# ZeningLin/ViBERTgrid-PyTorch

Hardware: AMD Instinct MI355X
Metric: training docs/sec, 512x512 img + seq_len 512, bert-base+resnet34; 1/2/4/8 GPU (higher is better)
Workload: dtype f32

## Files before the change

vibertgrid-pytorch_amd/csrc/gemm_planes.hip:

```cpp
#include "vbg_common.h"
#include <type_traits>
#include <cstdlib>
#include <hip/hip_ext.h>
#include "../../include/vbg.h"

namespace vbg {

typedef unsigned pg_u32x4 __attribute__((ext_vector_type(4)));
typedef __bf16 pg_bf16x8 __attribute__((ext_vector_type(8)));
constexpr unsigned PG_INVALID = 0x80000000u;

__device__ __forceinline__ __amdgpu_buffer_rsrc_t pg_rsrc(const void* base) {
    return __builtin_amdgcn_make_buffer_rsrc(const_cast<void*>(base), 0, (int)0x80000000u, 0x00020000);
}

typedef _Float16 pg_f16x8 __attribute__((ext_vector_type(8)));
__device__ __forceinline__ void pg_split2(float a, float b, unsigned& hi, unsigned& lo) {
    typedef float f32x2_t __attribute__((ext_vector_type(2)));
    typedef _Float16 f16x2_t __attribute__((ext_vector_type(2)));
    const f32x2_t v = {a, b};
    const f16x2_t h = __builtin_convertvector(v, f16x2_t);
    const f16x2_t l = __builtin_convertvector((v - __builtin_convertvector(h, f32x2_t)) * 2048.f, f16x2_t);
    hi = __builtin_bit_cast(unsigned, h);
    lo = __builtin_bit_cast(unsigned, l);
// ... 386 lines not shown
        if (gm >= M || gn >= N) continue;
        float4 v = *reinterpret_cast<const float4*>(&Ct[row * CTS + c]);
        if (add_bias) {
            const float4 b = *reinterpret_cast<const float4*>(bias + gn);
            v.x += b.x; v.y += b.y; v.z += b.z; v.w += b.w;
        }
        float* cp = C + (long long)gm * ldc + gn;
        if (atomic) {
            unsafeAtomicAdd(cp + 0, v.x); unsafeAtomicAdd(cp + 1, v.y); unsafeAtomicAdd(cp + 2, v.z); unsafeAtomicAdd(cp + 3, v.w);
            continue;
        }
        if (accumulate) {
            const float4 o = *reinterpret_cast<const float4*>(cp);
            v.x += o.x; v.y += o.y; v.z += o.z; v.w += o.w;
        }
        if (epi == VBG_EPI_RELU) v = make_float4(fmaxf(v.x, 0.f), fmaxf(v.y, 0.f), fmaxf(v.z, 0.f), fmaxf(v.w, 0.f));
        if (epi == VBG_EPI_MUL_GELU_GRAD) {
            const float4 hv = *reinterpret_cast<const float4*>(C2 + (long long)gm * ldc + gn);
            v.x *= gelu_erf_grad(hv.x); v.y *= gelu_erf_grad(hv.y); v.z *= gelu_erf_grad(hv.z); v.w *= gelu_erf_grad(hv.w);
        }
        if (C) *reinterpret_cast<float4*>(cp) = v;
        vmax = fmaxf(fmaxf(vmax, fmaxf(fabsf(v.x), fabsf(v.y))), fmaxf(fabsf(v.z), fabsf(v.w)));
        if (p.colsum) *reinterpret_cast<float4*>(&Ct[row * CTS + c]) = v;
        if (epi == VBG_EPI_GELU_DUAL) {
            v = make_float4(gelu_erf(v.x), gelu_erf(v.y), gelu_erf(v.z), gelu_erf(v.w));
            if (C2) *reinterpret_cast<float4*>(C2 + (long long)gm * ldc + gn) = v;
        }
        if (Cp) {
            const float e[4] = {v.x, v.y, v.z, v.w};
            unsigned short h[4], m[4], l[4];
#pragma unroll
            for (int t = 0; t < 4; ++t) {
                const unsigned u = __float_as_uint(e[t]);
                const float r1 = e[t] - __uint_as_float(u & 0xffff0000u);
                const unsigned u1 = __float_as_uint(r1);
                const float r2 = r1 - __uint_as_float(u1 & 0xffff0000u);
                h[t] = (unsigned short)(u >> 16); m[t] = (unsigned short)(u1 >> 16); l[t] = (unsigned short)(__float_as_uint(r2) >> 16);
            }
            unsigned short* o = Cp + (long long)gm * p.ldp + gn;
            *reinterpret_cast<uint2*>(o) = make_uint2(h[0] | ((unsigned)h[1] << 16), h[2] | ((unsigned)h[3] << 16));
            *reinterpret_cast<uint2*>(o + p.c_plane) = make_uint2(m[0] | ((unsigned)m[1] << 16), m[2] | ((unsigned)m[3] << 16));
            *reinterpret_cast<uint2*>(o + 2 * p.c_plane) = make_uint2(l[0] | ((unsigned)l[1] << 16), l[2] | ((unsigned)l[3] << 16));
        }
        if (Cq) {
            unsigned short* o = Cq + (long long)gm * p.ldq + gn;
            uint2 h, l;
            pg_split2(v.x * qsc, v.y * qsc, h.x, l.x);
            pg_split2(v.z * qsc, v.w * qsc, h.y, l.y);
            *reinterpret_cast<uint2*>(o) = h;
            *reinterpret_cast<uint2*>(o + p.q_plane) = l;
        }
    }
    if (p.colsum) {
        __syncthreads();
        if (tid < BN && n0 + tid < N) {
            float cs = 0.f;
            const int rows = min(BM, M - m0);
            for (int r = 0; r < rows; ++r) cs += Ct[r * CTS + tid];
            unsafeAtomicAdd(p.colsum + n0 + tid, cs);
        }
    }
    if (p.c_amax) {
        __syncthreads();
        vbg_amax_publish(vmax, p.c_amax, Ct);
    }
}

__device__ __forceinline__ void pg_split3(float x, unsigned short& h, unsigned short& m, unsigned short& l);

__global__ __launch_bounds__(512) void plane_gemm_256_kernel(const vbg_plane_gemm_desc p) {
    constexpr int BM = 256, BN = 256, WGN = 4, NW = 8, NT = 512, NST = 3, BK = 16;
    constexpr int WM = 128, WN = 64, TM = 4, TN = 2;
    constexpr int PA = BM * 32, PB = BN * 32;
    constexpr int STAGE = 3 * (PA + PB);
    constexpr int NIA = 3, NIB = 3;
    constexpr int CTS = BN + 4;
    constexpr int SMEM = NST * STAGE;
    static_assert(64 * CTS * 4 <= SMEM, "epilogue pass fits");
    __shared__ __attribute__((aligned(1024))) unsigned char smem[SMEM];

    const int tid = threadIdx.x, lane = tid & 63, wave = tid >> 6;
    const int M = p.M, N = p.N;
    const long long a_plane = p.a_plane, b_plane = p.b_plane, lda = p.lda, ldb = p.ldb;
    constexpr unsigned XCDS = 8, XCD_GROUP = 8;
    const unsigned gx = gridDim.x, gy = gridDim.y;
    const unsigned lin = blockIdx.x + gridDim.x * blockIdx.y;
    const unsigned total = gx * gy;
    const unsigned xcd = lin % XCDS, local = lin / XCDS;
    const unsigned per_xcd = (total + XCDS - 1) / XCDS, tall = (total % XCDS) ? (total % XCDS) : XCDS;
    const unsigned rem = xcd < tall ? xcd * per_xcd + local : tall * per_xcd + (xcd - tall) * (per_xcd - 1) + local;
    const unsigned band = XCD_GROUP * gy, bid = rem / band, first = bid * XCD_GROUP;
    const unsigned bm = min(gx - first, XCD_GROUP), inb = rem - bid * band;
    const unsigned tile_m = first + inb % bm, tile_n = inb / bm;
    const int m0 = (int)tile_m * BM, n0 = (int)tile_n * BN;
    if (m0 >= M || n0 >= N) return;
    const int ntiles = p.K / BK;

    unsigned avo[NIA], bvo[NIB];
    int alds[NIA], blds[NIB];
    {
        const int lrow = lane >> 1;
#pragma unroll
        for (int i = 0; i < NIA; ++i) {
            const int u = wave + NW * i, q = u / 8, rb = u % 8;
            const int r = rb * 32 + lrow;
            const int half = (lane & 1) ^ ((r >> 3) & 1);
            avo[i] = (m0 + r < M) ? (unsigned)(((long long)q * a_plane + (long long)r * lda) * 2 + half * 16) : PG_INVALID;
            alds[i] = __builtin_amdgcn_readfirstlane(q * PA + rb * 1024);
        }
#pragma unroll
        for (int i = 0; i < NIB; ++i) {
            const int u = wave + NW * i, q = u / 8, rb = u % 8;
            const int r = rb * 32 + lrow;
            const int half = (lane & 1) ^ ((r >> 3) & 1);
            bvo[i] = (n0 + r < N) ? (unsigned)(((long long)q * b_plane + (long long)r * ldb) * 2 + half * 16) : PG_INVALID;
            blds[i] = __builtin_amdgcn_readfirstlane(3 * PA + q * PB + rb * 1024);
        }
    }
    const unsigned short* abase = p.A + (long long)m0 * lda;
    const unsigned short* bbase = p.B + (long long)n0 * ldb;
    typedef __attribute__((address_space(3))) void* lds_ptr;
    auto issue = [&](int stage, unsigned inv) {
        unsigned char* sb = smem + stage * STAGE;
        const __amdgpu_buffer_rsrc_t ra = pg_rsrc(abase), rb = pg_rsrc(bbase);
#pragma unroll
        for (int i = 0; i < NIA; ++i)
            __builtin_amdgcn_raw_ptr_buffer_load_lds(ra, (lds_ptr)(sb + alds[i]), 16, (int)(avo[i] | inv), 0, 0, 0);
#pragma unroll
        for (int i = 0; i < NIB; ++i)
            __builtin_amdgcn_raw_ptr_buffer_load_lds(rb, (lds_ptr)(sb + blds[i]), 16, (int)(bvo[i] | inv), 0, 0, 0);
        abase += BK;
        bbase += BK;
    };

    const int wm = wave / WGN, wn = wave % WGN;
    const int lr = lane & 31, lk = lane >> 5;
    const int fo = lr * 32 + ((lk ^ ((lr >> 3) & 1)) << 4);
    f32x16 acc[TM][TN];
#pragma unroll
    for (int i = 0; i < TM; ++i)
#pragma unroll
        for (int j = 0; j < TN; ++j)
#pragma unroll
            for (int r = 0; r < 16; ++r) acc[i][j][r] = 0.f;
    pg_u32x4 fa[3][TM], fb[3][TN];
    auto read_frags = [&](int stage) {
        const unsigned char* as = smem + stage * STAGE + (wm * WM) * 32 + fo;
        const unsigned char* bs = smem + stage * STAGE + 3 * PA + (wn * WN) * 32 + fo;
        constexpr int order[3] = {2, 0, 1};
#pragma unroll
        for (int o = 0; o < 3; ++o) {
            const int q = order[o];
#pragma unroll
            for (int i = 0; i < TM; ++i) fa[q][i] = *reinterpret_cast<const pg_u32x4*>(as + q * PA + i * 32 * 32);
#pragma unroll
            for (int j = 0; j < TN; ++j) fb[q][j] = *reinterpret_cast<const pg_u32x4*>(bs + q * PB + j * 32 * 32);
        }
    };
    auto mma = [&]() {
        constexpr int qa[6] = {2, 0, 1, 1, 0, 0}, qb[6] = {0, 2, 1, 0, 1, 0};
#pragma unroll
        for (int t = 0; t < 6; ++t)
#pragma unroll
            for (int i = 0; i < TM; ++i)
#pragma unroll
                for (int j = 0; j < TN; ++j)
                    acc[i][j] = __builtin_amdgcn_mfma_f32_32x32x16_bf16(__builtin_bit_cast(pg_bf16x8, fa[qa[t]][i]),
                                                                        __builtin_bit_cast(pg_bf16x8, fb[qb[t]][j]), acc[i][j], 0, 0, 0);
    };
    constexpr int NIW = NIA + NIB;
    issue(0, 0u);
    issue(1, ntiles > 1 ? 0u : PG_INVALID);
    asm volatile("s_waitcnt vmcnt(%0)" ::"n"(NIW) : "memory");
    __builtin_amdgcn_s_barrier();
    int cur = 0;
    for (int t = 0; t < ntiles; ++t) {
        const int nxt = (cur + 1 == NST) ? 0 : cur + 1;
        const int nn = (nxt + 1 == NST) ? 0 : nxt + 1;
        issue(nn, t + 2 < ntiles ? 0u : PG_INVALID);
        read_frags(cur);
        mma();
        asm volatile("s_waitcnt vmcnt(%0) lgkmcnt(0)" ::"n"(NIW) : "memory");
        __builtin_amdgcn_s_barrier();
        cur = nxt;
    }
    __syncthreads();

    const float* bias = p.bias;
    const int epi = p.epi;
    const float alpha = p.alpha;
    const long long ldc = p.ldc;
    float* const C = p.C;
    float* const C2 = p.C2;
    unsigned short* const Cp = p.Cp;
    float* const Ct = reinterpret_cast<float*>(smem);
    constexpr int QN = BN / 4;
#pragma unroll
    for (int ps = 0; ps < 4; ++ps) {
        if (wm == (ps >> 1)) {
#pragma unroll
            for (int ii = 0; ii < 2; ++ii)
#pragma unroll
                for (int j = 0; j < TN; ++j)
#pragma unroll
                    for (int r = 0; r < 16; ++r)
                        Ct[(ii * 32 + (r & 3) + 8 * (r >> 2) + 4 * lk) * CTS + wn * WN + j * 32 + lr] = acc[2 * (ps & 1) + ii][j][r] * alpha;
        }
        __syncthreads();
#pragma unroll
        for (int q = 0; q < 64 * QN / NT; ++q) {
            const int idx = tid + q * NT;
            const int row = idx / QN, c = (idx % QN) * 4;
            const int gm = m0 + ps * 64 + row, gn = n0 + c;
            if (gm >= M || gn >= N) continue;
            float4 v = *reinterpret_cast<const float4*>(&Ct[row * CTS + c]);
            if (bias) {
                const float4 b = *reinterpret_cast<const float4*>(bias + gn);
                v.x += b.x; v.y += b.y; v.z += b.z; v.w += b.w;
            }
            float* cp = C + (long long)gm * ldc + gn;
            if (epi == VBG_EPI_RELU) v = make_float4(fmaxf(v.x, 0.f), fmaxf(v.y, 0.f), fmaxf(v.z, 0.f), fmaxf(v.w, 0.f));
            if (epi == VBG_EPI_MUL_GELU_GRAD) {
                const float4 hv = *reinterpret_cast<const float4*>(C2 + (long long)gm * ldc + gn);
                v.x *= gelu_erf_grad(hv.x); v.y *= gelu_erf_grad(hv.y); v.z *= gelu_erf_grad(hv.z); v.w *= gelu_erf_grad(hv.w);
            }
            if (C) *reinterpret_cast<float4*>(cp) = v;
            if (epi == VBG_EPI_GELU_DUAL) {
                v = make_float4(gelu_erf(v.x), gelu_erf(v.y), gelu_erf(v.z), gelu_erf(v.w));
                if (C2) *reinterpret_cast<float4*>(C2 + (long long)gm * ldc + gn) = v;
            }
            if (Cp) {
                const float e[4] = {v.x, v.y, v.z, v.w};
                unsigned short h[4], m[4], l[4];
#pragma unroll
                for (int t = 0; t < 4; ++t) pg_split3(e[t], h[t], m[t], l[t]);
                unsigned short* o = Cp + (long long)gm * p.ldp + gn;
                *reinterpret_cast<uint2*>(o) = make_uint2(h[0] | ((unsigned)h[1] << 16), h[2] | ((unsigned)h[3] << 16));
                *reinterpret_cast<uint2*>(o + p.c_plane) = make_uint2(m[0] | ((unsigned)m[1] << 16), m[2] | ((unsigned)m[3] << 16));
                *reinterpret_cast<uint2*>(o + 2 * p.c_plane) = make_uint2(l[0] | ((unsigned)l[1] << 16), l[2] | ((unsigned)l[3] << 16));
            }
        }
        __syncthreads();
    }
}

__device__ __forceinline__ void pg_split3(float x, unsigned short& h, unsigned short& m, unsigned short& l) {
    const unsigned u = __float_as_uint(x);
    const float r1 = x - __uint_as_float(u & 0xffff0000u);
    const unsigned u1 = __float_as_uint(r1);
    const float r2 = r1 - __uint_as_float(u1 & 0xffff0000u);
    h = (unsigned short)(u >> 16); m = (unsigned short)(u1 >> 16); l = (unsigned short)(__float_as_uint(r2) >> 16);
}

__global__ __launch_bounds__(256) void split_planes_kernel(const float* __restrict__ x, long long ldx, int rows, int cols,
                                                            unsigned short* __restrict__ out, int ldp, long long plane, int relu,
                                                            float* colsum) {
    extern __shared__ float sh_cols[];
    const int cpr = ldp / 8;
    const long long n = (long long)rows * cpr;
    const long long stride = (long long)gridDim.x * blockDim.x;
    float cs[8] = {0.f, 0.f, 0.f, 0.f, 0.f, 0.f, 0.f, 0.f};
    const long long i0 = (long long)blockIdx.x * blockDim.x + threadIdx.x;
    for (long long i = i0; i < n; i += stride) {
        const int r = (int)(i / cpr), c = (int)(i % cpr) * 8;
        float e[8];
        if (c + 8 <= cols && ((ldx & 3) == 0) && ((((uintptr_t)x) & 15) == 0)) {
            const float4 a = *reinterpret_cast<const float4*>(x + (long long)r * ldx + c);
            const float4 b = *reinterpret_cast<const float4*>(x + (long long)r * ldx + c + 4);
            e[0] = a.x; e[1] = a.y; e[2] = a.z; e[3] = a.w; e[4] = b.x; e[5] = b.y; e[6] = b.z; e[7] = b.w;
        } else {
#pragma unroll
            for (int t = 0; t < 8; ++t) e[t] = (c + t < cols) ? x[(long long)r * ldx + c + t] : 0.f;
        }
        unsigned short h[8], m[8], l[8];
#pragma unroll
        for (int t = 0; t < 8; ++t) {
            cs[t] += e[t];
            pg_split3(relu ? fmaxf(e[t], 0.f) : e[t], h[t], m[t], l[t]);
        }
        unsigned short* o = out + (long long)r * ldp + c;
        auto pack = [](const unsigned short* s) {
            return make_uint4(s[0] | ((unsigned)s[1] << 16), s[2] | ((unsigned)s[3] << 16), s[4] | ((unsigned)s[5] << 16), s[6] | ((unsigned)s[7] << 16));
        };
        *reinterpret_cast<uint4*>(o) = pack(h);
        *reinterpret_cast<uint4*>(o + plane) = pack(m);
        *reinterpret_cast<uint4*>(o + 2 * plane) = pack(l);
    }
    if (colsum) {
        for (int c = threadIdx.x; c < ldp; c += blockDim.x) sh_cols[c] = 0.f;
        __syncthreads();
        if (i0 < n) {
            const int c = (int)(i0 % cpr) * 8;
#pragma unroll
            for (int t = 0; t < 8; ++t) atomicAdd(&sh_cols[c + t], cs[t]);
        }
        __syncthreads();
        for (int c = threadIdx.x; c < cols; c += blockDim.x) {
            const float v = sh_cols[c];
            if (v != 0.f) unsafeAtomicAdd(colsum + c, v);
        }
    }
}

__global__ __launch_bounds__(256) void split_planes_pair_kernel(const float* __restrict__ x, long long ldx, int rows, int cols,
                                                                 unsigned short* __restrict__ out, int ldp, long long plane,
                                                                 const unsigned* amax, float* colsum) {
    extern __shared__ float sh_cols[];
    const float sc = amax ? vbg_pow2_scale(vbg_amax_read(amax)).x : 1.f;
    float cs[8] = {0.f, 0.f, 0.f, 0.f, 0.f, 0.f, 0.f, 0.f};
    const long long i0 = (long long)blockIdx.x * blockDim.x + threadIdx.x;
    const int cpr = ldp / 8;
    const long long n = (long long)rows * cpr;
    const long long stride = (long long)gridDim.x * blockDim.x;
    const bool vec = ((ldx & 3) == 0) && ((((uintptr_t)x) & 15) == 0);
    for (long long i = (long long)blockIdx.x * blockDim.x + threadIdx.x; i < n; i += stride) {
        const int r = (int)(i / cpr), c = (int)(i % cpr) * 8;
        float e[8];
        if (c + 8 <= cols && vec) {
            const float4 a = *reinterpret_cast<const float4*>(x + (long long)r * ldx + c);
            const float4 b = *reinterpret_cast<const float4*>(x + (long long)r * ldx + c + 4);
            e[0] = a.x; e[1] = a.y; e[2] = a.z; e[3] = a.w; e[4] = b.x; e[5] = b.y; e[6] = b.z; e[7] = b.w;
        } else {
#pragma unroll
            for (int t = 0; t < 8; ++t) e[t] = (c + t < cols) ? x[(long long)r * ldx + c + t] : 0.f;
        }
#pragma unroll
        for (int t = 0; t < 8; ++t) { cs[t] += e[t]; e[t] *= sc; }
        uint4 h, l;
        pg_split2(e[0], e[1], h.x, l.x); pg_split2(e[2], e[3], h.y, l.y); pg_split2(e[4], e[5], h.z, l.z); pg_split2(e[6], e[7], h.w, l.w);
        unsigned short* o = out + (long long)r * ldp + c;
        *reinterpret_cast<uint4*>(o) = h;
        *reinterpret_cast<uint4*>(o + plane) = l;
    }
    if (colsum) {
        for (int c = threadIdx.x; c < ldp; c += blockDim.x) sh_cols[c] = 0.f;
        __syncthreads();
        if (i0 < n) {
            const int c = (int)(i0 % cpr) * 8;
#pragma unroll
            for (int t = 0; t < 8; ++t) atomicAdd(&sh_cols[c + t], cs[t]);
        }
        __syncthreads();
        for (int c = threadIdx.x; c < cols; c += blockDim.x) {
            const float v = sh_cols[c];
            if (v != 0.f) unsafeAtomicAdd(colsum + c, v);
        }
    }
}

__global__ __launch_bounds__(256) void col_l1_max_kernel(const vbg_l1_entry* __restrict__ tab, unsigned* __restrict__ out) {
    const vbg_l1_entry e = tab[blockIdx.y];
    const int c0 = blockIdx.x * 64;
    if (c0 >= e.cols) return;
    const int tx = threadIdx.x & 15, ty = threadIdx.x >> 4;
    const int c = c0 + tx * 4;
    const bool vec = (e.ld & 3) == 0 && ((((uintptr_t)e.w) & 15) == 0) && c + 4 <= e.cols;
    float4 s = make_float4(0.f, 0.f, 0.f, 0.f);
#pragma unroll 4
    for (int r = ty; r < e.rows; r += 16) {
        const float* p = e.w + (long long)r * e.ld + c;
        if (vec) {
            const float4 v = *reinterpret_cast<const float4*>(p);
            s.x += fabsf(v.x); s.y += fabsf(v.y); s.z += fabsf(v.z); s.w += fabsf(v.w);
        } else {
            if (c < e.cols) s.x += fabsf(p[0]);
            if (c + 1 < e.cols) s.y += fabsf(p[1]);
            if (c + 2 < e.cols) s.z += fabsf(p[2]);
            if (c + 3 < e.cols) s.w += fabsf(p[3]);
        }
    }
    __shared__ float4 red[16][16];
    red[ty][tx] = s;
    __syncthreads();
    if (ty == 0) {
        float4 t = red[0][tx];
#pragma unroll
        for (int g = 1; g < 16; ++g) { const float4 v = red[g][tx]; t.x += v.x; t.y += v.y; t.z += v.z; t.w += v.w; }
        float m = fmaxf(fmaxf(t.x, t.y), fmaxf(t.z, t.w));
#pragma unroll
        for (int o = 8; o > 0; o >>= 1) m = fmaxf(m, __shfl_xor(m, o, 64));
        if (tx == 0) atomicMax(out + blockIdx.y, __float_as_uint(m));
    }
}

__global__ __launch_bounds__(256) void split_planes_t_kernel(const float* __restrict__ x, long long ldx, int rows, int cols,
                                                              unsigned short* __restrict__ out, int ldp, long long plane) {
    __shared__ float t[64][65];
    const int r0 = blockIdx.x * 64, c0 = blockIdx.y * 64;
    const int tid = threadIdx.x;
    const bool vec = ((ldx & 3) == 0) && ((((uintptr_t)x) & 15) == 0);
#pragma unroll
    for (int i = 0; i < 4; ++i) {
        const int f = tid + i * 256, r = f / 16, c = (f % 16) * 4;
        float4 v = make_float4(0.f, 0.f, 0.f, 0.f);
        if (r0 + r < rows) {
            const float* src = x + (long long)(r0 + r) * ldx + c0 + c;
            if (vec && c0 + c + 4 <= cols) v = *reinterpret_cast<const float4*>(src);
            else {
                if (c0 + c + 0 < cols) v.x = src[0];
                if (c0 + c + 1 < cols) v.y = src[1];
                if (c0 + c + 2 < cols) v.z = src[2];
                if (c0 + c + 3 < cols) v.w = src[3];
            }
        }
        t[r][c] = v.x; t[r][c + 1] = v.y; t[r][c + 2] = v.z; t[r][c + 3] = v.w;
    }
    __syncthreads();
#pragma unroll
    for (int i = 0; i < 2; ++i) {
        const int f = tid + i * 256, c = f / 8, rg = (f % 8) * 8;
        if (c0 + c >= cols || r0 + rg >= ldp) continue;
        unsigned short h[8], m[8], l[8];
#pragma unroll
        for (int e = 0; e < 8; ++e) pg_split3(t[rg + e][c], h[e], m[e], l[e]);
        unsigned short* o = out + (long long)(c0 + c) * ldp + r0 + rg;
        auto pack = [](const unsigned short* s) {
            return make_uint4(s[0] | ((unsigned)s[1] << 16), s[2] | ((unsigned)s[3] << 16), s[4] | ((unsigned)s[5] << 16), s[6] | ((unsigned)s[7] << 16));
        };
        *reinterpret_cast<uint4*>(o) = pack(h);
        *reinterpret_cast<uint4*>(o + plane) = pack(m);
        *reinterpret_cast<uint4*>(o + 2 * plane) = pack(l);
    }
}

template <bool PAIR>
__global__ __launch_bounds__(256) void split_planes_t_batched_kernel(const float* __restrict__ src, unsigned short* __restrict__ dst,
                                                                      const long long* __restrict__ tbl, int njobs, long long plane) {
    __shared__ float t[64][65];
    int j = 0;
    while (j + 1 < njobs && (long long)blockIdx.x >= tbl[(j + 1) * 6 + 5]) ++j;
    const long long* e = tbl + j * 6;
    const float* x = src + e[0];
    const int rows = (int)e[1], cols = (int)e[2], ldp = (int)e[4];
    unsigned short* out = dst + e[3];
    const int local = (int)(blockIdx.x - e[5]);
    const int tr = (ldp + 63) / 64;
    const int r0 = (local % tr) * 64, c0 = (local / tr) * 64;
    const int tid = threadIdx.x;
    const long long ldx = cols;
#pragma unroll
    for (int i = 0; i < 4; ++i) {
        const int f = tid + i * 256, r = f / 16, c = (f % 16) * 4;
        float v[4] = {0.f, 0.f, 0.f, 0.f};
        if (r0 + r < rows) {
#pragma unroll
            for (int q = 0; q < 4; ++q)
                if (c0 + c + q < cols) v[q] = x[(long long)(r0 + r) * ldx + c0 + c + q];
        }
        t[r][c] = v[0]; t[r][c + 1] = v[1]; t[r][c + 2] = v[2]; t[r][c + 3] = v[3];
    }
    __syncthreads();
#pragma unroll
    for (int i = 0; i < 2; ++i) {
        const int f = tid + i * 256, c = f / 8, rg = (f % 8) * 8;
        if (c0 + c >= cols || r0 + rg >= ldp) continue;
        unsigned short* o = out + (long long)(c0 + c) * ldp + r0 + rg;
        if constexpr (PAIR) {
            uint4 h, l;
            pg_split2(t[rg + 0][c], t[rg + 1][c], h.x, l.x); pg_split2(t[rg + 2][c], t[rg + 3][c], h.y, l.y);
            pg_split2(t[rg + 4][c], t[rg + 5][c], h.z, l.z); pg_split2(t[rg + 6][c], t[rg + 7][c], h.w, l.w);
            *reinterpret_cast<uint4*>(o) = h;
            *reinterpret_cast<uint4*>(o + plane) = l;
            continue;
        }
        unsigned short h[8], m[8], l[8];
#pragma unroll
        for (int q = 0; q < 8; ++q) pg_split3(t[rg + q][c], h[q], m[q], l[q]);
        auto pack = [](const unsigned short* s) {
            return make_uint4(s[0] | ((unsigned)s[1] << 16), s[2] | ((unsigned)s[3] << 16), s[4] | ((unsigned)s[5] << 16), s[6] | ((unsigned)s[7] << 16));
        };
        *reinterpret_cast<uint4*>(o) = pack(h);
        *reinterpret_cast<uint4*>(o + plane) = pack(m);
        *reinterpret_cast<uint4*>(o + 2 * plane) = pack(l);
    }
}

template <int BM, int BN, int WGM, int WGN, int NST, bool TRANS = false, int FORM = 1>
static void pg_launch_pair(const vbg_plane_gemm_desc& d, hipStream_t s, hipEvent_t e0, hipEvent_t e1) {
    dim3 g(cdiv(d.M, BM), cdiv(d.N, BN), 1);
    if (d.ngroups > 0) {
        int total = 0;
        for (int i = 0; i < d.ngroups; ++i) total += d.grp[i].tiles_m * d.grp[i].tiles_n;
        g = dim3(total, 1, 1);
    }
    (void)hipGetLastError();
    if (e0 && e1) hipExtLaunchKernelGGL((plane_gemm_kernel<BM, BN, WGM, WGN, NST, TRANS, FORM>), g, dim3(WGM * WGN * 64), 0, s, e0, e1, 0, d);
    else hipLaunchKernelGGL((plane_gemm_kernel<BM, BN, WGM, WGN, NST, TRANS, FORM>), g, dim3(WGM * WGN * 64), 0, s, d);
}

template <int BM, int BN, int WGM, int WGN, int NST, bool TRANS = false>
static void pg_launch(const vbg_plane_gemm_desc& d, hipStream_t s, hipEvent_t e0, hipEvent_t e1) {
    dim3 g(cdiv(d.M, BM), cdiv(d.N, BN), d.splitk);
    if (d.ngroups > 0) {
        int total = 0;
        for (int i = 0; i < d.ngroups; ++i) total += d.grp[i].tiles_m * d.grp[i].tiles_n;
        g = dim3(total, 1, d.splitk);
    }
    (void)hipGetLastError();
    if (e0 && e1) hipExtLaunchKernelGGL((plane_gemm_kernel<BM, BN, WGM, WGN, NST, TRANS>), g, dim3(WGM * WGN * 64), 0, s, e0, e1, 0, d);
    else hipLaunchKernelGGL((plane_gemm_kernel<BM, BN, WGM, WGN, NST, TRANS>), g, dim3(WGM * WGN * 64), 0, s, d);
}

}

using namespace vbg;

static int plane_gemm_dispatch(const vbg_plane_gemm_desc* desc, void* stream, void* e0, void* e1) {
    VBG_CHECK_ARG(desc != nullptr);
    vbg_plane_gemm_desc d = *desc;
    if (d.ngroups > 0) {
        VBG_CHECK_ARG(d.ngroups <= VBG_PLANE_MAX_GROUPS && d.Cp == nullptr && d.bias == nullptr && d.C2 == nullptr);
        for (int i = 0; i < d.ngroups; ++i) {
            vbg_plane_group& g = d.grp[i];
            VBG_CHECK_ARG(g.A && g.B && g.C && g.M > 0 && g.N > 0 && g.N % 4 == 0 && g.ldc % 4 == 0 && ((uintptr_t)g.C & 15) == 0);
            VBG_CHECK_ARG(((uintptr_t)g.A & 15) == 0 && ((uintptr_t)g.B & 15) == 0 && g.a_plane % 8 == 0 && g.b_plane % 8 == 0);
            if (d.trans) VBG_CHECK_ARG(g.lda % 32 == 0 && g.ldb % 32 == 0 && g.lda >= g.M && g.ldb >= g.N);
            else VBG_CHECK_ARG(g.lda % 8 == 0 && g.ldb % 8 == 0 && g.lda >= d.K && g.ldb >= d.K);
            VBG_CHECK_ARG(2 * g.a_plane * 2 + 256 * g.lda * 2 < 0x7fffffffll && 2 * g.b_plane * 2 + 256 * g.ldb * 2 < 0x7fffffffll);
            const int bn = (d.trans || d.tile != 64064) ? 128 : 64, bm = (d.trans && d.tile == 256128) ? 256 : bn;
            g.tiles_m = (g.M + bm - 1) / bm;
            g.tiles_n = (g.N + bn - 1) / bn;
        }
        d.A = d.grp[0].A; d.B = d.grp[0].B; d.C = d.grp[0].C; d.M = d.grp[0].M; d.N = d.grp[0].N;
        d.a_plane = d.grp[0].a_plane; d.b_plane = d.grp[0].b_plane; d.lda = d.grp[0].lda; d.ldb = d.grp[0].ldb; d.ldc = d.grp[0].ldc;
        if (!d.trans && d.tile != 64064) d.tile = 128129;
    }
    VBG_CHECK_ARG(d.A && d.B && (d.C || d.Cp || d.Cq));
    if (d.cq_ref_in) VBG_CHECK_ARG(d.Cq && d.cq_mul > 0.f && d.tile != 256256 && !d.trans && d.ngroups == 0 && d.splitk == 1);
    VBG_CHECK_ARG(d.M >= 0 && d.N >= 0 && d.K > 0);
    if (d.trans) VBG_CHECK_ARG(d.lda % 32 == 0 && d.ldb % 32 == 0 && d.lda >= d.M && d.ldb >= d.N);
    else VBG_CHECK_ARG(d.K % 32 == 0 && d.lda % 8 == 0 && d.ldb % 8 == 0 && d.lda >= d.K && d.ldb >= d.K);
    VBG_CHECK_ARG(((uintptr_t)d.A & 15) == 0 && ((uintptr_t)d.B & 15) == 0 && (d.a_plane % 8) == 0 && (d.b_plane % 8) == 0);
    VBG_CHECK_ARG(d.N % 4 == 0 && d.ldc % 4 == 0 && ((uintptr_t)d.C & 15) == 0 && ((uintptr_t)d.C2 & 15) == 0 && ((uintptr_t)d.bias & 15) == 0);
    VBG_CHECK_ARG(2 * d.a_plane * 2 + (long long)256 * d.lda * 2 < 0x7fffffffll && 2 * d.b_plane * 2 + (long long)256 * d.ldb * 2 < 0x7fffffffll);
    if (d.splitk < 1) d.splitk = 1;
    if (d.splitk > 1) VBG_CHECK_ARG(d.accumulate == 1 && d.C);
    if (d.accumulate) VBG_CHECK_ARG(d.epi == VBG_EPI_NONE && d.Cp == nullptr);
    if (d.colsum) VBG_CHECK_ARG(d.splitk == 1 && d.ngroups == 0 && !d.trans && !d.accumulate && d.epi != VBG_EPI_GELU_DUAL && d.tile != 256256);
    if (d.c_amax) VBG_CHECK_ARG(d.tile != 256256 && !d.trans && d.ngroups == 0 && d.splitk == 1);
    if (d.epi == VBG_EPI_GELU_DUAL) VBG_CHECK_ARG(d.C2 != nullptr || d.Cp != nullptr || d.Cq != nullptr);
    if (d.epi == VBG_EPI_MUL_GELU_GRAD) VBG_CHECK_ARG(d.C2 != nullptr && d.ngroups == 0 && !d.trans);
    if (d.Cp) VBG_CHECK_ARG(d.ldp % 8 == 0 && d.ldp >= d.N && ((uintptr_t)d.Cp & 7) == 0 && d.c_plane % 4 == 0);
    if (d.Cq) VBG_CHECK_ARG(d.ldq % 8 == 0 && d.ldq >= d.N && ((uintptr_t)d.Cq & 7) == 0 && d.q_plane % 4 == 0 && !d.accumulate && d.ngroups == 0 &&
                            !d.trans && d.tile != 256256);
    if (d.M == 0 || d.N == 0) return VBG_OK;
    hipStream_t s = (hipStream_t)stream;
    int tile = d.tile;
    if (d.form == 1 || d.form == 2) {
        VBG_CHECK_ARG(d.splitk == 1 && (d.ngroups == 0 || d.trans));
        hipEvent_t ev0 = (hipEvent_t)e0, ev1 = (hipEvent_t)e1;
        if (d.form == 2) {
            if (d.trans) {
                if (tile == 256128) pg_launch_pair<256, 128, 4, 2, 3, true, 2>(d, s, ev0, ev1);
                else pg_launch_pair<128, 128, 4, 2, 3, true, 2>(d, s, ev0, ev1);
            } else if (tile == 256128) pg_launch_pair<256, 128, 4, 2, 3, false, 2>(d, s, ev0, ev1);
            else if (tile == 128129 || tile == 0) pg_launch_pair<128, 128, 4, 2, 4, false, 2>(d, s, ev0, ev1);
            else if ((tile == 64064 || tile == 64004) && d.ngroups == 0 && !d.c_amax && !d.cq_ref_in && !d.colsum) {
                if (tile == 64004) pg_launch_pair<64, 64, 2, 2, 4, false, 2>(d, s, ev0, ev1);
                else pg_launch_pair<64, 64, 2, 2, 3, false, 2>(d, s, ev0, ev1);
            }
            else return VBG_EARG;
            VBG_LAUNCH_RET();
        }
        if (d.trans) {
            if (tile == 256128) pg_launch_pair<256, 128, 4, 2, 3, true>(d, s, ev0, ev1);
            else pg_launch_pair<128, 128, 4, 2, 3, true>(d, s, ev0, ev1);
            VBG_LAUNCH_RET();
        }
        if (tile == 256128) pg_launch_pair<256, 128, 4, 2, 3>(d, s, ev0, ev1);
        else if (tile == 128130) pg_launch_pair<128, 128, 2, 4, 3>(d, s, ev0, ev1);
        else if (tile == 128129 || tile == 0) pg_launch_pair<128, 128, 4, 2, 4>(d, s, ev0, ev1);
        else if ((tile == 64064 || tile == 64004) && d.ngroups == 0 && !d.c_amax && !d.cq_ref_in && !d.colsum) {
            if (tile == 64004) pg_launch_pair<64, 64, 2, 2, 4>(d, s, ev0, ev1);
            else pg_launch_pair<64, 64, 2, 2, 3>(d, s, ev0, ev1);
        } else return VBG_EARG;
        VBG_LAUNCH_RET();
    }
    VBG_CHECK_ARG(d.form == 0);
    if (d.trans) {
        if (tile == 256128) pg_launch<256, 128, 4, 2, 2, true>(d, s, (hipEvent_t)e0, (hipEvent_t)e1);
        else if (tile == 128130) pg_launch<128, 128, 2, 4, 3, true>(d, s, (hipEvent_t)e0, (hipEvent_t)e1);
        else pg_launch<128, 128, 4, 2, 3, true>(d, s, (hipEvent_t)e0, (hipEvent_t)e1);
        VBG_LAUNCH_RET();
    }
    if (tile == 0) {
        const long t128 = (long)cdiv(d.M, 128) * cdiv(d.N, 128) * d.splitk;
        tile = (t128 >= 200 && d.N >= 128) ? 128128 : 64064;
    }
    if (tile == 256256) {
        VBG_CHECK_ARG(d.splitk == 1 && !d.accumulate && d.K % 16 == 0);
        const dim3 g(cdiv(d.M, 256), cdiv(d.N, 256));
        (void)hipGetLastError();
        hipEvent_t ev0 = (hipEvent_t)e0, ev1 = (hipEvent_t)e1;
        if (ev0 && ev1) hipExtLaunchKernelGGL(plane_gemm_256_kernel, g, dim3(512), 0, s, ev0, ev1, 0, d);
        else hipLaunchKernelGGL(plane_gemm_256_kernel, g, dim3(512), 0, s, d);
        VBG_LAUNCH_RET();
    }
    if (tile == 256128) pg_launch<256, 128, 4, 2, 2>(d, s, (hipEvent_t)e0, (hipEvent_t)e1);
    else if (tile == 128128) pg_launch<128, 128, 2, 2, 3>(d, s, (hipEvent_t)e0, (hipEvent_t)e1);
    else if (tile == 128129) pg_launch<128, 128, 4, 2, 3>(d, s, (hipEvent_t)e0, (hipEvent_t)e1);
    else if (tile == 128130) pg_launch<128, 128, 2, 4, 3>(d, s, (hipEvent_t)e0, (hipEvent_t)e1);
    else if (tile == 128064) pg_launch<128, 64, 2, 2, 3>(d, s, (hipEvent_t)e0, (hipEvent_t)e1);
    else if (tile == 64064) pg_launch<64, 64, 2, 2, 3>(d, s, (hipEvent_t)e0, (hipEvent_t)e1);
    else return VBG_EARG;
    VBG_LAUNCH_RET();
}

extern "C" int vbg_plane_gemm(const vbg_plane_gemm_desc* desc, void* stream) { return plane_gemm_dispatch(desc, stream, nullptr, nullptr); }

extern "C" int vbg_plane_gemm_timed(const vbg_plane_gemm_desc* desc, void* stream, void* start_event, void* stop_event) {
    VBG_CHECK_ARG(start_event && stop_event);
    return plane_gemm_dispatch(desc, stream, start_event, stop_event);
}

extern "C" int vbg_split_planes(const float* x, long long ldx, int rows, int cols, unsigned short* out, int ldp, long long plane,
                                int relu, float* colsum_accum, void* stream) {
    VBG_CHECK_ARG(rows >= 0 && cols >= 0 && ldp % 32 == 0 && ldp >= cols && plane >= (long long)rows * ldp && plane % 8 == 0);
    if (rows == 0 || cols == 0) return VBG_OK;
    VBG_CHECK_ARG(x && out && ((uintptr_t)out & 15) == 0);
    const long long n = (long long)rows * (ldp / 8);
    long long g = (n + 255) / 256;
    size_t lds = 0;
    if (colsum_accum) {
        VBG_CHECK_ARG(relu == 0 && ldp * 4 <= 64 * 1024);
        const long long cpr = ldp / 8;
        long long a = cpr, b = 256;
        while (b) { const long long t = a % b; a = b; b = t; }
        const long long unit = cpr / a;
        long long k = 288 / unit;
        if (k < 1) k = 1;
        const long long need = (g + unit - 1) / unit;
        if (k > need) k = need;
        g = k * unit;
        lds = (size_t)ldp * 4;
    } else if (g > 256 * 16) {
        g = 256 * 16;
    }
    VBG_LAUNCH(split_planes_kernel, dim3((unsigned)g), dim3(256), lds, (hipStream_t)stream, x, ldx, rows, cols, out, ldp, plane, relu,
               colsum_accum);
    VBG_LAUNCH_RET();
}

extern "C" int vbg_split_planes_pair(const float* x, long long ldx, int rows, int cols, unsigned short* out, int ldp, long long plane,
                                     const unsigned* amax, float* colsum_accum, void* stream) {
    VBG_CHECK_ARG(rows >= 0 && cols >= 0 && ldp % 32 == 0 && ldp >= cols && plane >= (long long)rows * ldp && plane % 8 == 0);
    if (rows == 0 || cols == 0) return VBG_OK;
    VBG_CHECK_ARG(x && out && ((uintptr_t)out & 15) == 0);
    const long long n = (long long)rows * (ldp / 8);
    long long g = (n + 255) / 256;
    size_t lds = 0;
    if (colsum_accum) {
        VBG_CHECK_ARG(ldp * 4 <= 64 * 1024);
        const long long cpr = ldp / 8;
        long long a = cpr, b = 256;
        while (b) { const long long t = a % b; a = b; b = t; }
        const long long unit = cpr / a;
        long long k = 288 / unit;
        if (k < 1) k = 1;
        const long long need = (g + unit - 1) / unit;
        if (k > need) k = need;
        g = k * unit;
        lds = (size_t)ldp * 4;
    } else if (g > 256 * 16) {
        g = 256 * 16;
    }
    VBG_LAUNCH(split_planes_pair_kernel, dim3((unsigned)g), dim3(256), lds, (hipStream_t)stream, x, ldx, rows, cols, out, ldp, plane, amax, colsum_accum);
    VBG_LAUNCH_RET();
}

extern "C" int vbg_col_l1_max(const vbg_l1_entry* table_dev, int n, int max_cols, unsigned* out, void* stream) {
    VBG_CHECK_ARG(n >= 0 && max_cols >= 0);
    if (n == 0 || max_cols == 0) return VBG_OK;
    VBG_CHECK_ARG(table_dev && out);
    VBG_LAUNCH(col_l1_max_kernel, dim3((unsigned)((max_cols + 63) / 64), (unsigned)n), dim3(256), 0, (hipStream_t)stream, table_dev, out);
    VBG_LAUNCH_RET();
}

extern "C" int vbg_split_planes_t(const float* x, long long ldx, int rows, int cols, unsigned short* out, int ldp, long long plane,
                                  void* stream) {
    VBG_CHECK_ARG(rows >= 0 && cols >= 0 && ldp % 32 == 0 && ldp >= rows && plane >= (long long)cols * ldp && plane % 8 == 0);
    if (rows == 0 || cols == 0) return VBG_OK;
    VBG_CHECK_ARG(x && out && ((uintptr_t)out & 15) == 0);
    VBG_LAUNCH(split_planes_t_kernel, dim3(cdiv(ldp, 64), cdiv(cols, 64)), dim3(256), 0, (hipStream_t)stream, x, ldx, rows, cols, out, ldp, plane);
    VBG_LAUNCH_RET();
}

extern "C" int vbg_split_planes_t_batched(const float* src, unsigned short* dst, const long long* tbl_dev, int njobs, int total_tiles,
                                          long long plane, void* stream) {
    VBG_CHECK_ARG(njobs >= 0 && total_tiles >= 0);
    if (njobs == 0 || total_tiles == 0) return VBG_OK;
    VBG_CHECK_ARG(src && dst && tbl_dev && ((uintptr_t)dst & 15) == 0 && plane % 8 == 0);
    VBG_LAUNCH(split_planes_t_batched_kernel<false>, dim3(total_tiles), dim3(256), 0, (hipStream_t)stream, src, dst, tbl_dev, njobs, plane);
    VBG_LAUNCH_RET();
}

extern "C" int vbg_split_planes_pair_t_batched(const float* src, unsigned short* dst, const long long* tbl_dev, int njobs, int total_tiles,
                                               long long plane, void* stream) {
    VBG_CHECK_ARG(njobs >= 0 && total_tiles >= 0);
    if (njobs == 0 || total_tiles == 0) return VBG_OK;
    VBG_CHECK_ARG(src && dst && tbl_dev && ((uintptr_t)dst & 15) == 0 && plane % 8 == 0);
    VBG_LAUNCH(split_planes_t_batched_kernel<true>, dim3(total_tiles), dim3(256), 0, (hipStream_t)stream, src, dst, tbl_dev, njobs, plane);
    VBG_LAUNCH_RET();
}
```

Before: 246.8.

## Tile split_planes_pair into 2D column-group/row-block grid with unrolled row walk

Rewrites the fp16-pair plane split kernel so each block owns a fixed column group (up to 32 x 8 columns) and a contiguous block of rows, with threads walking rows four at a time. This replaces the grid-stride loop with per-element div/mod. It also replaces the whole-row shared-memory column-sum reduction with a fixed 256-entry one. The launcher sizes row blocks so the colsum path has about 144 row blocks, cutting global atomics while keeping parallelism. The risk is less parallelism for small inputs and larger per-thread register use from the 4-row unroll.

```diff
diff --git a/vibertgrid-pytorch_amd/csrc/gemm_planes.hip b/vibertgrid-pytorch_amd/csrc/gemm_planes.hip
--- a/vibertgrid-pytorch_amd/csrc/gemm_planes.hip
+++ b/vibertgrid-pytorch_amd/csrc/gemm_planes.hip
@@ -712,49 +712,66 @@
     }
 }
 
+template <bool VEC, int N>
+__device__ __forceinline__ void pair_rows(const float* __restrict__ x, long long ldx, int cols, unsigned short* __restrict__ out, int ldp,
+                                          long long plane, float sc, int c, int r, int rstep, float (&cs)[8]) {
+    float e[N][8];
+#pragma unroll
+    for (int u = 0; u < N; ++u) {
+        const float* p = x + (long long)(r + u * rstep) * ldx + c;
+        if constexpr (VEC) {
+            const float4 a = *reinterpret_cast<const float4*>(p);
+            const float4 b = *reinterpret_cast<const float4*>(p + 4);
+            e[u][0] = a.x; e[u][1] = a.y; e[u][2] = a.z; e[u][3] = a.w; e[u][4] = b.x; e[u][5] = b.y; e[u][6] = b.z; e[u][7] = b.w;
+        } else {
+#pragma unroll
+            for (int t = 0; t < 8; ++t) e[u][t] = (c + t < cols) ? p[t] : 0.f;
+        }
+    }
+#pragma unroll
+    for (int u = 0; u < N; ++u) {
+#pragma unroll
+        for (int t = 0; t < 8; ++t) { cs[t] += e[u][t]; e[u][t] *= sc; }
+        uint4 h, l;
+        pg_split2(e[u][0], e[u][1], h.x, l.x); pg_split2(e[u][2], e[u][3], h.y, l.y);
+        pg_split2(e[u][4], e[u][5], h.z, l.z); pg_split2(e[u][6], e[u][7], h.w, l.w);
+        unsigned short* o = out + (long long)(r + u * rstep) * ldp + c;
+        *reinterpret_cast<uint4*>(o) = h;
+        *reinterpret_cast<uint4*>(o + plane) = l;
+    }
+}
+template <bool VEC>
+__device__ __forceinline__ void pair_walk(const float* __restrict__ x, long long ldx, int cols, unsigned short* __restrict__ out, int ldp,
+                                          long long plane, float sc, int c, int r, int r_end, int rstep, float (&cs)[8]) {
+    for (; r + 3 * rstep < r_end; r += 4 * rstep) pair_rows<VEC, 4>(x, ldx, cols, out, ldp, plane, sc, c, r, rstep, cs);
+    for (; r < r_end; r += rstep) pair_rows<VEC, 1>(x, ldx, cols, out, ldp, plane, sc, c, r, rstep, cs);
+}
+
 __global__ __launch_bounds__(256) void split_planes_pair_kernel(const float* __restrict__ x, long long ldx, int rows, int cols,
                                                                  unsigned short* __restrict__ out, int ldp, long long plane,
-                                                                 const unsigned* amax, float* colsum) {
-    extern __shared__ float sh_cols[];
+                                                                 const unsigned* amax, float* colsum, int cwl, int rpb) {
+    __shared__ float sh_cols[256];
     const float sc = amax ? vbg_pow2_scale(vbg_amax_read(amax)).x : 1.f;
     float cs[8] = {0.f, 0.f, 0.f, 0.f, 0.f, 0.f, 0.f, 0.f};
-    const long long i0 = (long long)blockIdx.x * blockDim.x + threadIdx.x;
-    const int cpr = ldp / 8;
-    const long long n = (long long)rows * cpr;
-    const long long stride = (long long)gridDim.x * blockDim.x;
-    const bool vec = ((ldx & 3) == 0) && ((((uintptr_t)x) & 15) == 0);
-    for (long long i = (long long)blockIdx.x * blockDim.x + threadIdx.x; i < n; i += stride) {
-        const int r = (int)(i / cpr), c = (int)(i % cpr) * 8;
-        float e[8];
-        if (c + 8 <= cols && vec) {
-            const float4 a = *reinterpret_cast<const float4*>(x + (long long)r * ldx + c);
-            const float4 b = *reinterpret_cast<const float4*>(x + (long long)r * ldx + c + 4);
-            e[0] = a.x; e[1] = a.y; e[2] = a.z; e[3] = a.w; e[4] = b.x; e[5] = b.y; e[6] = b.z; e[7] = b.w;
-        } else {
-#pragma unroll
-            for (int t = 0; t < 8; ++t) e[t] = (c + t < cols) ? x[(long long)r * ldx + c + t] : 0.f;
-        }
-#pragma unroll
-        for (int t = 0; t < 8; ++t) { cs[t] += e[t]; e[t] *= sc; }
-        uint4 h, l;
-        pg_split2(e[0], e[1], h.x, l.x); pg_split2(e[2], e[3], h.y, l.y); pg_split2(e[4], e[5], h.z, l.z); pg_split2(e[6], e[7], h.w, l.w);
-        unsigned short* o = out + (long long)r * ldp + c;
-        *reinterpret_cast<uint4*>(o) = h;
-        *reinterpret_cast<uint4*>(o + plane) = l;
+    const int cpr = ldp / 8, cw = 1 << cwl, rstep = 256 >> cwl;
+    const int ncg = (cpr + cw - 1) >> cwl;
+    const int cg = (int)(blockIdx.x % (unsigned)ncg), rg = (int)(blockIdx.x / (unsigned)ncg);
+    const int cl = threadIdx.x & (cw - 1);
+    const int c = (cg * cw + cl) * 8;
+    const int r0 = rg * rpb + (int)(threadIdx.x >> cwl), r_end = (int)min((long long)rows, ((long long)rg + 1) * rpb);
+    if (colsum) sh_cols[threadIdx.x] = 0.f;
+    if (c < ldp) {
+        if (((ldx & 3) == 0) && ((((uintptr_t)x) & 15) == 0) && c + 8 <= cols) pair_walk<true>(x, ldx, cols, out, ldp, plane, sc, c, r0, r_end, rstep, cs);
+        else pair_walk<false>(x, ldx, cols, out, ldp, plane, sc, c, r0, r_end, rstep, cs);
     }
     if (colsum) {
-        for (int c = threadIdx.x; c < ldp; c += blockDim.x) sh_cols[c] = 0.f;
         __syncthreads();
-        if (i0 < n) {
-            const int c = (int)(i0 % cpr) * 8;
-#pragma unroll
-            for (int t = 0; t < 8; ++t) atomicAdd(&sh_cols[c + t], cs[t]);
-        }
+#pragma unroll
+        for (int t = 0; t < 8; ++t) atomicAdd(&sh_cols[cl * 8 + t], cs[t]);
         __syncthreads();
-        for (int c = threadIdx.x; c < cols; c += blockDim.x) {
-            const float v = sh_cols[c];
-            if (v != 0.f) unsafeAtomicAdd(colsum + c, v);
-        }
+        const int cc = cg * cw * 8 + (int)threadIdx.x;
+        const float v = sh_cols[threadIdx.x];
+        if ((int)threadIdx.x < cw * 8 && cc < cols && v != 0.f) unsafeAtomicAdd(colsum + cc, v);
     }
 }
 
@@ -1056,25 +1073,20 @@
     VBG_CHECK_ARG(rows >= 0 && cols >= 0 && ldp % 32 == 0 && ldp >= cols && plane >= (long long)rows * ldp && plane % 8 == 0);
     if (rows == 0 || cols == 0) return VBG_OK;
     VBG_CHECK_ARG(x && out && ((uintptr_t)out & 15) == 0);
-    const long long n = (long long)rows * (ldp / 8);
-    long long g = (n + 255) / 256;
-    size_t lds = 0;
+    const int cpr = ldp / 8;
+    int cwl = 5;
+    while ((1 << cwl) > cpr) --cwl;
+    const long long rstep = 256 >> cwl, ncg = (cpr + (1 << cwl) - 1) >> cwl;
+    long long rpb = 4 * rstep;
     if (colsum_accum) {
         VBG_CHECK_ARG(ldp * 4 <= 64 * 1024);
-        const long long cpr = ldp / 8;
-        long long a = cpr, b = 256;
-        while (b) { const long long t = a % b; a = b; b = t; }
-        const long long unit = cpr / a;
-        long long k = 288 / unit;
-        if (k < 1) k = 1;
-        const long long need = (g + unit - 1) / unit;
-        if (k > need) k = need;
-        g = k * unit;
-        lds = (size_t)ldp * 4;
-    } else if (g > 256 * 16) {
-        g = 256 * 16;
-    }
-    VBG_LAUNCH(split_planes_pair_kernel, dim3((unsigned)g), dim3(256), lds, (hipStream_t)stream, x, ldx, rows, cols, out, ldp, plane, amax, colsum_accum);
+        const long long need = (((long long)rows + 143) / 144 + rpb - 1) / rpb * rpb;
+        if (need > rpb) rpb = need;
+    }
+    const long long g = (((long long)rows + rpb - 1) / rpb) * ncg;
+    VBG_CHECK_ARG(g <= 0x7fffffffLL && rpb <= 0x7fffffffLL);
+    VBG_LAUNCH(split_planes_pair_kernel, dim3((unsigned)g), dim3(256), 0, (hipStream_t)stream, x, ldx, rows, cols, out, ldp, plane, amax, colsum_accum,
+               cwl, (int)rpb);
     VBG_LAUNCH_RET();
 }
 
```

Result: slower. 236.7 (-4.1%).
